# SciSharp/Gym.NET

Hardware: AMD Instinct MI355X
Metric: env-steps/sec (higher is better)
Workload: dtype f32

## Files before the change

### gym.net_amd/csrc/envs.hpp

```cpp
#pragma once
#include <hip/hip_runtime.h>
#include <stdint.h>

#include "philox.hpp"

namespace gymnet {


typedef float f2 __attribute__((ext_vector_type(2)));
namespace vm {
__device__ __forceinline__ float splat(float, float v) { return v; }
__device__ __forceinline__ f2 splat(f2, float v) { return f2{v, v}; }
__device__ __forceinline__ float fma(float a, float b, float c) { return fmaf(a, b, c); }
__device__ __forceinline__ f2 fma(f2 a, f2 b, f2 c) { return __builtin_elementwise_fma(a, b, c); }
template <class T> __device__ __forceinline__ T fmak(float k, T b, T c) { return fma(splat(b, k), b, c); }
template <class T> __device__ __forceinline__ T fmac(T a, T b, float k) { return fma(a, b, splat(a, k)); }
}

__device__ __forceinline__ void sincos_quadrant(float s, float c, float n, float &s_out, float &c_out) {
    const uint32_t q = (uint32_t)(int)n;
    const uint32_t q30 = q << 30, q31 = q << 31;
    const bool odd = (int32_t)q31 < 0;
    const float ss = odd ? c : s, cc = odd ? s : c;
    s_out = __uint_as_float(__builtin_amdgcn_bitop3_b32(__float_as_uint(ss), q30, 0x80000000u, 0x78));
// ... 39 lines not shown
    T ps = vm::fmac(vm::splat(z, -1.9515295891e-4f), z, 8.3321608736e-3f);
    ps = vm::fmac(ps, z, -1.6666654611e-1f);
    const T s = vm::fma(r * z, ps, r);
    T pc = vm::fmac(vm::splat(z, 2.443315711809948e-5f), z, -1.388731625493765e-3f);
    pc = vm::fmac(pc, z, 4.166664568298827e-2f);
    pc = vm::fmac(pc, z, -0.5f);
    const T c = vm::fmac(pc, z, 1.0f);
    if constexpr (sizeof(T) == sizeof(float)) {
        sincos_quadrant(s, c, n, s_out, c_out);
    } else {
        float s0, c0, s1, c1;
        sincos_quadrant(s.x, c.x, n.x, s0, c0);
        sincos_quadrant(s.y, c.y, n.y, s1, c1);
        s_out = T{s0, s1};
        c_out = T{c0, c1};
    }
}

constexpr float kSmallAngle = 0.785f;
__device__ __forceinline__ void sincos_tiny(float x, float &s_out, float &c_out) {
    const float z = x * x;
    float ps = fmaf(-1.9515295891e-4f, z, 8.3321608736e-3f);
    ps = fmaf(ps, z, -1.6666654611e-1f);
    s_out = fmaf(x * z, ps, x);
    float pc = fmaf(2.443315711809948e-5f, z, -1.388731625493765e-3f);
    pc = fmaf(pc, z, 4.166664568298827e-2f);
    c_out = fmaf(z * z, pc, fmaf(-0.5f, z, 1.0f));
}

template <bool BOUNDED = false>
__device__ __forceinline__ void sincos_f32(float x, float &s_out, float &c_out) {
    if constexpr (!BOUNDED) {
        if (__builtin_expect(fabsf(x) > 65536.0f, 0)) {
            sincosf(x, &s_out, &c_out);
            return;
        }
    }
    sincos_bounded<float>(x, s_out, c_out);
}
__device__ __forceinline__ float sin_f32(float x) { float s, c; sincos_f32(x, s, c); return s; }
__device__ __forceinline__ float cos_f32(float x) { float s, c; sincos_f32(x, s, c); return c; }

template <typename Dummy = void>
struct DivByTotalMass {
    static constexpr float C = 0.1f + 1.0f;
    static constexpr float ZH = 1.0f / C;
    static constexpr float ZL = (float)(1.0 / (double)C - (double)ZH);
    __device__ __forceinline__ static float apply(float x) { return fmaf(x, ZH, x * ZL); }
};

struct CartPole {
    static constexpr int S = 4;
    static constexpr int O = 4;
    static constexpr bool OBS_ALIASES_STATE = true;
    static constexpr bool HAS_SBD = true;
    static constexpr bool BOX_ACTION = false;
    static constexpr bool PACKED2 = false;
    static constexpr bool PIPE_LANES = false, PIPE_PAIRS = false;
    using Action = int32_t;
    using Real = float;
    static constexpr bool RESET_TAKES_KEY = false;
    static constexpr const char *NAME = "CartPole";
    static constexpr int32_t ACTION_N = 2;

    static constexpr float gravity = 9.8f;
    static constexpr float masspole = 0.1f;
    static constexpr float total_mass = 0.1f + 1.0f;
    static constexpr float length = 0.5f;
    static constexpr float polemass_length = 0.1f * 0.5f;
    static constexpr float force_mag = 10.0f;
    static constexpr float tau = 0.02f;
    static constexpr float theta_threshold = 0.20943951606750488f;
    static constexpr float x_threshold = 2.4f;

    __device__ __forceinline__ static float div_tm(float x) { return DivByTotalMass<>::apply(x); }

    static constexpr bool HAS_SMALL_ANGLE_PATH = true;
    static constexpr int ANGLE_ROW = 2;
    static constexpr float SMALL_ANGLE_BOUND = kSmallAngle;

    template <bool SMALL_ANGLE = false, bool AUTORESET = false>
    __device__ __forceinline__ static void step(float (&s)[S], Action a, float &reward, bool &done) {
        const float x = s[0], x_dot = s[1], theta = s[2], theta_dot = s[3];
        const float force = (a == 1) ? force_mag : -force_mag;
        float sintheta, costheta;
        if constexpr (SMALL_ANGLE) sincos_tiny(theta, sintheta, costheta);
        else sincos_f32(theta, sintheta, costheta);
        const float temp = div_tm(force + polemass_length * theta_dot * theta_dot * sintheta);
        const float thetaacc = (gravity * sintheta - costheta * temp)
                               / (length * (4.0f / 3.0f - div_tm(masspole * costheta * costheta)));
        const float xacc = temp - div_tm(polemass_length * thetaacc * costheta);
        const float nx = x + tau * x_dot;
        const float nx_dot = x_dot + tau * xacc;
        const float ntheta = theta + tau * theta_dot;
        const float ntheta_dot = theta_dot + tau * thetaacc;
        s[0] = nx; s[1] = nx_dot; s[2] = ntheta; s[3] = ntheta_dot;
        const double vx = __builtin_fma((double)tau, (double)x_dot, (double)x);
        const double vtheta = __builtin_fma((double)tau, (double)theta_dot, (double)theta);
        done = __builtin_fabs(vx) > (double)x_threshold || __builtin_fabs(vtheta) > (double)theta_threshold;
        reward = 1.0f;
    }

    __device__ __forceinline__ static void reset(float (&s)[S], const PhiloxWords &r) {
#pragma unroll
        for (int k = 0; k < 4; ++k) s[k] = -0.05f + 0.1f * u01_24(r.w[k]);
    }

    __device__ __forceinline__ static void observe(const float (&s)[S], float (&o)[O]) {
#pragma unroll
        for (int k = 0; k < 4; ++k) o[k] = s[k];
    }
    __device__ __forceinline__ static void observe_fresh(const float (&s)[S], float (&o)[O]) { observe(s, o); }
    __device__ __forceinline__ static void step_observe(float (&s)[S], Action a, float &reward, bool &done, float (&o)[O]) {
        step(s, a, reward, done);
        observe(s, o);
    }
};

struct Pendulum {
    static constexpr int S = 2;
    static constexpr int O = 3;
    static constexpr bool OBS_ALIASES_STATE = false;
    static constexpr int OBS_ROW_OF_STATE[S] = {-1, 2};
    static constexpr bool HAS_SBD = false;
    static constexpr bool BOX_ACTION = true;
    static constexpr bool PACKED2 = false;
    static constexpr bool PIPE_LANES = false, PIPE_PAIRS = false;
    static constexpr bool HAS_SMALL_ANGLE_PATH = false;
    using Action = float;
    using Real = float;
    static constexpr bool RESET_TAKES_KEY = false;
    static constexpr const char *NAME = "Pendulum";
    static constexpr float ACTION_LOW = -2.0f, ACTION_HIGH = 2.0f;
    static constexpr float PI = 3.14159265358979323846f;

    __device__ __forceinline__ static float fmod_2pi(float a) {
        constexpr float m = 2.0f * PI, inv_m = 1.0f / m;
        const float ax = fabsf(a);
        if (__builtin_expect(!(ax < 4194304.0f * m), 0)) return fmodf(a, m);
        float q = truncf(ax * inv_m);
        float r = fmaf(-q, m, ax);
        q = r < 0.0f ? q - 1.0f : (r >= m ? q + 1.0f : q);
        r = fmaf(-q, m, ax);
        return copysignf(r, a);
    }

    __device__ __forceinline__ static float floored_mod_2pi(float a) {
        float r = fmod_2pi(a);
        if (r < 0.0f) r += 2.0f * PI;
        return r;
    }

    __device__ __forceinline__ static void step(float (&s)[S], Action a, float &reward, bool &done) {
        const float max_speed = 8.0f, max_torque = 2.0f, dt = 0.05f;
        const float th = s[0], thdot = s[1];
        const float u = a < -max_torque ? -max_torque : (a > max_torque ? max_torque : a);
        const float nrm = floored_mod_2pi(th + PI) - PI;
        const float costs = nrm * nrm + 0.1f * (thdot * thdot) + 0.001f * (u * u);
        float newthdot = thdot + (15.0f * sin_f32(th) + 3.0f * u) * dt;
        newthdot = newthdot < -max_speed ? -max_speed : (newthdot > max_speed ? max_speed : newthdot);
        const float newth = th + newthdot * dt;
        s[0] = newth; s[1] = newthdot;
        reward = -costs;
        done = false;
    }

    __device__ __forceinline__ static void reset(float (&s)[S], const PhiloxWords &r) {
        s[0] = -PI + (2.0f * PI) * u01_24(r.w[0]);
        s[1] = -1.0f + 2.0f * u01_24(r.w[1]);
    }

    __device__ __forceinline__ static void observe(const float (&s)[S], float (&o)[O]) {
        float sn, cs;
        sincos_f32(s[0], sn, cs);
        o[0] = cs; o[1] = sn; o[2] = s[1];
    }
    __device__ __forceinline__ static void observe_fresh(const float (&s)[S], float (&o)[O]) { observe(s, o); }
    __device__ __forceinline__ static void step_observe(float (&s)[S], Action a, float &reward, bool &done, float (&o)[O]) {
        step(s, a, reward, done);
        observe(s, o);
    }
};

// ... 225 lines not shown
```

### gym.net_amd/csrc/lanes.hpp

```cpp
#pragma once
#include <hip/hip_runtime.h>
#include <stdint.h>

namespace gymnet {

template <class T, int N> struct VecOf { typedef T type __attribute__((ext_vector_type(N))); };
typedef float f32x4 __attribute__((ext_vector_type(4)));
typedef int32_t i32x4 __attribute__((ext_vector_type(4)));

template <class T, int VEC>
constexpr int piece_of() { return (int)(16 / sizeof(T)) < VEC ? (int)(16 / sizeof(T)) : VEC; }

template <class T, int VEC, bool NT, bool GUARD>
__device__ __forceinline__ void load_row(const T *__restrict__ p, int64_t i0, int64_t n, T (&v)[VEC]) {
    if constexpr (VEC > 1 && sizeof(T) > 1) {
        if (!GUARD || i0 + VEC <= n) {
            constexpr int P = piece_of<T, VEC>();
            static_assert(VEC % P == 0, "VEC must be a whole number of 16-byte pieces");
            typedef typename VecOf<T, P>::type V;
#pragma unroll
            for (int q = 0; q < VEC / P; ++q) {
                V t;
                if constexpr (NT) t = __builtin_nontemporal_load(reinterpret_cast<const V *>(p + i0 + q * P));
                else t = *reinterpret_cast<const V *>(p + i0 + q * P);
#pragma unroll
                for (int j = 0; j < P; ++j) v[q * P + j] = t[j];
            }
            return;
        }
    }
#pragma unroll
    for (int j = 0; j < VEC; ++j) {
        if (!GUARD || i0 + j < n) { if constexpr (NT) v[j] = __builtin_nontemporal_load(p + i0 + j); else v[j] = p[i0 + j]; }
        else v[j] = T(0);
    }
}

template <class T, int VEC, bool NT, bool GUARD>
__device__ __forceinline__ void store_row(T *__restrict__ p, int64_t i0, int64_t n, const T (&v)[VEC]) {
    if constexpr (VEC > 1 && sizeof(T) > 1) {
        if (!GUARD || i0 + VEC <= n) {
            constexpr int P = piece_of<T, VEC>();
            static_assert(P == 2 || P == 4, "16-byte pieces of 4- or 8-byte elements");
            typedef typename VecOf<T, P>::type V;
#pragma unroll
            for (int q = 0; q < VEC / P; ++q) {
                V t;
                if constexpr (P == 4) t = V{v[q * P], v[q * P + 1], v[q * P + 2], v[q * P + 3]};
                else t = V{v[q * P], v[q * P + 1]};
#ifdef GYMNET_PROBE_STORE_SC1
                if constexpr (NT && sizeof(T) == 4 && P == 4) {
                    asm volatile("global_store_dwordx4 %0, %1, off sc1" :: "v"(p + i0 + q * P), "v"(t) : "memory");
                    continue;
                }
#endif
                if constexpr (NT) __builtin_nontemporal_store(t, reinterpret_cast<V *>(p + i0 + q * P));
                else *reinterpret_cast<V *>(p + i0 + q * P) = t;
            }
            return;
        }
    }
#pragma unroll
    for (int j = 0; j < VEC; ++j)
        if (!GUARD || i0 + j < n) { if constexpr (NT) __builtin_nontemporal_store(v[j], p + i0 + j); else p[i0 + j] = v[j]; }
}

template <int VEC, bool NT, bool GUARD>
__device__ __forceinline__ void store_u8(uint8_t *__restrict__ p, int64_t i0, int64_t n, const uint8_t (&v)[VEC]) {
    if constexpr (VEC == 2) {
        if (!GUARD || i0 + 2 <= n) {
            const uint16_t w = (uint16_t)((uint16_t)v[0] | ((uint16_t)v[1] << 8));
            if constexpr (NT) __builtin_nontemporal_store(w, reinterpret_cast<uint16_t *>(p + i0));
            else *reinterpret_cast<uint16_t *>(p + i0) = w;
            return;
        }
    }
    if constexpr (VEC == 4) {
        if (!GUARD || i0 + 4 <= n) {
            const uint32_t w = (uint32_t)v[0] | ((uint32_t)v[1] << 8) | ((uint32_t)v[2] << 16) | ((uint32_t)v[3] << 24);
            if constexpr (NT) __builtin_nontemporal_store(w, reinterpret_cast<uint32_t *>(p + i0));
            else *reinterpret_cast<uint32_t *>(p + i0) = w;
            return;
        }
    }
#pragma unroll
    for (int j = 0; j < VEC; ++j)
        if (!GUARD || i0 + j < n) { if constexpr (NT) __builtin_nontemporal_store(v[j], p + i0 + j); else p[i0 + j] = v[j]; }
}

template <int VEC, bool NT, bool GUARD>
__device__ __forceinline__ void load_f32(const float *__restrict__ p, int64_t i0, int64_t n, float (&v)[VEC]) { load_row<float, VEC, NT, GUARD>(p, i0, n, v); }
template <int VEC, bool NT, bool GUARD>
__device__ __forceinline__ void store_f32(float *__restrict__ p, int64_t i0, int64_t n, const float (&v)[VEC]) { store_row<float, VEC, NT, GUARD>(p, i0, n, v); }
template <int VEC, bool NT, bool GUARD>
__device__ __forceinline__ void load_i32(const int32_t *__restrict__ p, int64_t i0, int64_t n, int32_t (&v)[VEC]) { load_row<int32_t, VEC, NT, GUARD>(p, i0, n, v); }
template <int VEC, bool NT, bool GUARD>
__device__ __forceinline__ void store_i32(int32_t *__restrict__ p, int64_t i0, int64_t n, const int32_t (&v)[VEC]) { store_row<int32_t, VEC, NT, GUARD>(p, i0, n, v); }

__device__ __forceinline__ uint32_t lane_id() {
    return __builtin_amdgcn_mbcnt_hi(~0u, __builtin_amdgcn_mbcnt_lo(~0u, 0u));
}

}
```

### gym.net_amd/csrc/step_kernels.hpp

```cpp
#pragma once
#include "kernels.hpp"

#include <cstdio>
#include <type_traits>

#include "lanes.hpp"
#include "philox.hpp"

namespace gymnet {

__device__ __forceinline__ float abs_real(float x) { return fabsf(x); }
__device__ __forceinline__ double abs_real(double x) { return __builtin_fabs(x); }

template <class Env, bool UNIFORM_KEY = false>
__device__ __forceinline__ void draw_reset(typename Env::Real (&s)[Env::S], uint64_t key, uint64_t lane, uint64_t tick) {
    if constexpr (Env::RESET_TAKES_KEY) Env::reset(s, key, lane, tick);
    else Env::reset(s, lane_words<UNIFORM_KEY>(key, lane, tick));
}

template <class Env>
__device__ __forceinline__ constexpr bool state_row_own(int k) {
    if constexpr (Env::OBS_ALIASES_STATE) return true; else return Env::OBS_ROW_OF_STATE[k] < 0;
}
template <class Env>
__device__ __forceinline__ const typename Env::Real *state_row_src(const typename Env::Real *state, int64_t state_stride,
                                                                    const typename Env::Real *obs_in, int64_t obs_stride, int k) {
    if constexpr (Env::OBS_ALIASES_STATE) return state + k * state_stride;
    else return Env::OBS_ROW_OF_STATE[k] < 0 ? state + k * state_stride : obs_in + Env::OBS_ROW_OF_STATE[k] * obs_stride;
}

__device__ __forceinline__ uint32_t wave_shard() {
    return (uint32_t)((((int64_t)blockIdx.x * blockDim.x + threadIdx.x) >> 6) & (kShards - 1));
}

template <int VEC, class Args>
__device__ __forceinline__ void count_after_done(const Args &a, const bool (&after)[VEC]) {
    uint32_t total = 0;
#pragma unroll
    for (int j = 0; j < VEC; ++j) total += (uint32_t)__popcll(__ballot(after[j]));
    if (total && lane_id() == (uint32_t)(__ffsll((unsigned long long)__ballot(1)) - 1))
        atomicAdd(&a.after_done[wave_shard() * kAfterStride], (unsigned long long)total);
}

template <class Env, bool AUTORESET, bool SMALL_ANGLE = false>
__device__ __forceinline__ void advance_sublane(typename Env::Real (&sj)[Env::S], typename Env::Action act, int32_t &sbd, float &rw,
                                                bool &dn, bool &after, bool in_range, typename Env::Real (&oj)[Env::O]) {
    if constexpr (Env::HAS_SMALL_ANGLE_PATH) Env::template step<SMALL_ANGLE, AUTORESET>(sj, act, rw, dn);
    else if constexpr (Env::OBS_ALIASES_STATE) Env::step(sj, act, rw, dn);
    else Env::step_observe(sj, act, rw, dn, oj);
    if constexpr (!AUTORESET && Env::HAS_SBD) {
        if (dn) {
            if (sbd == -1) { sbd = 0; }
            else { after = in_range; sbd += 1; rw = 0.0f; }
        }
    }
}

template <class Env, int VEC>
__device__ __forceinline__ bool wave_angles_small(const typename Env::Real (&s)[Env::S][VEC]) {
    if constexpr (!Env::HAS_SMALL_ANGLE_PATH) return false;
    else {
        bool small = true;
#pragma unroll
        for (int j = 0; j < VEC; ++j) small = small && (abs_real(s[Env::ANGLE_ROW][j]) <= Env::SMALL_ANGLE_BOUND);
        return __ballot(!small) == 0;
    }
}

template <class Env, int VEC, bool AUTORESET, bool GUARD, bool PACK = true>
__device__ __forceinline__ void advance_all(typename Env::Real (&s)[Env::S][VEC], typename Env::Action (&act)[VEC], int32_t (&sbd)[VEC],
                                            float (&rw)[VEC], bool (&dn)[VEC], bool (&after)[VEC], typename Env::Real (&o)[Env::O][VEC],
                                            int64_t i0, int64_t n) {
    constexpr int S = Env::S, O = Env::O;
    using Real = typename Env::Real;
#ifndef GYMNET_PROBE_NO_PACK
    constexpr bool kPack = true;
#else
    constexpr bool kPack = false;
#endif
    if constexpr (Env::PACKED2 && VEC == 2 && kPack && PACK) {
        Env::step_observe_x2(s, act, rw, dn, o);
    } else {
        auto all_sublanes = [&](auto small_tag) {
#pragma unroll
            for (int j = 0; j < VEC; ++j) {
                Real sj[S], oj[O];
#pragma unroll
                for (int k = 0; k < S; ++k) sj[k] = s[k][j];
                advance_sublane<Env, AUTORESET, decltype(small_tag)::value>(sj, act[j], sbd[j], rw[j], dn[j], after[j], !GUARD || i0 + j < n, oj);
#pragma unroll
                for (int k = 0; k < S; ++k) s[k][j] = sj[k];
                if constexpr (!Env::OBS_ALIASES_STATE) {
#pragma unroll
                    for (int k = 0; k < O; ++k) o[k][j] = oj[k];
                }
            }
        };
        if constexpr (Env::HAS_SMALL_ANGLE_PATH) {
            if (wave_angles_small<Env, VEC>(s)) all_sublanes(std::true_type{});
            else all_sublanes(std::false_type{});
        } else {
            all_sublanes(std::false_type{});
        }
    }
}

template <class Env, int VEC, bool LANE_SEEDS>
__device__ __forceinline__ void reset_pending(uint32_t pending, typename Env::Real (&s)[Env::S][VEC], typename Env::Real (&o)[Env::O][VEC],
                                              const StepArgsT<typename Env::Real> &a, int64_t i0, int64_t n, uint64_t tick) {
    constexpr int S = Env::S, O = Env::O;
    using Real = typename Env::Real;
    while (pending) {
        const int j = __ffs(pending) - 1;
        pending &= pending - 1;
        Real sj[S];
        bool drawn = false;
        if constexpr (LANE_SEEDS) {
            if (a.lane_seed) {
                draw_reset<Env, false>(sj, i0 + j < n ? a.lane_seed[i0 + j] : a.seed, a.lane_offset + (uint64_t)(i0 + j), tick);
                drawn = true;
            }
        }
        if (!drawn) draw_reset<Env, true>(sj, a.seed, a.lane_offset + (uint64_t)(i0 + j), tick);
        Real oj[O];
        if constexpr (!Env::OBS_ALIASES_STATE) Env::observe_fresh(sj, oj);
#pragma unroll
        for (int jj = 0; jj < VEC; ++jj) {
            if (jj == j) {
#pragma unroll
                for (int k = 0; k < S; ++k) s[k][jj] = sj[k];
                if constexpr (!Env::OBS_ALIASES_STATE) {
#pragma unroll
                    for (int k = 0; k < O; ++k) o[k][jj] = oj[k];
                }
            }
        }
    }
}

template <class Env>
constexpr bool has_split_reset() { return Env::RESET_TAKES_KEY && Env::OBS_ALIASES_STATE; }

__device__ __forceinline__ PhiloxWords neighbour_words(const PhiloxWords &w) {
    PhiloxWords o;
#pragma unroll
    for (int k = 0; k < 4; ++k) o.w[k] = (uint32_t)__builtin_amdgcn_mov_dpp((int)w.w[k], 0xB1, 0xF, 0xF, true);
    return o;
}

#ifdef GYMNET_PROBE_RESET_MASKED
constexpr bool kResetFullExec = false;
#else
constexpr bool kResetFullExec = true;
#endif

template <class Env>
struct ResetScratch {
    uint32_t slot[64];
    typename Env::Real draw[64][Env::S];
};

__device__ __forceinline__ void wave_lds_fence() {
    __builtin_amdgcn_fence(__ATOMIC_RELEASE, "wavefront");
    __builtin_amdgcn_wave_barrier();
    __builtin_amdgcn_fence(__ATOMIC_ACQUIRE, "wavefront");
}

template <class Env, int VEC, bool LANE_SEEDS>
__device__ __forceinline__ void reset_pending_wave(uint32_t pending, typename Env::Real (&s)[Env::S][VEC], const StepArgsT<typename Env::Real> &a,
                                                   int64_t i0, int64_t n, uint64_t tick, ResetScratch<Env> *sc) {
    constexpr int S = Env::S;
    using Real = typename Env::Real;
    static_assert(Env::OBS_ALIASES_STATE, "the compacted reset hands back the state only");
    const uint32_t lane = lane_id();
    uint32_t rank[VEC];
    uint32_t total = 0;
#pragma unroll
    for (int j = 0; j < VEC; ++j) {
        const uint64_t m = __ballot((pending >> j) & 1u);
        rank[j] = total + __builtin_amdgcn_mbcnt_hi((uint32_t)(m >> 32), __builtin_amdgcn_mbcnt_lo((uint32_t)m, 0u));
        total += (uint32_t)__popcll(m);
    }
    if (total == 0) return;
    const int64_t wave_i0 = i0 - (int64_t)lane * VEC;
    constexpr bool SPLIT = has_split_reset<Env>();
    const uint32_t active = (uint32_t)__popcll(__ballot(1));
    const uint32_t A = SPLIT ? active >> 1 : active;
    if constexpr (SPLIT) {
        if (A == 0) {
            Real o_unused[Env::O][VEC];
            reset_pending<Env, VEC, LANE_SEEDS>(pending, s, o_unused, a, i0, n, tick);
            return;
        }
    }
    for (uint32_t base = 0; base < total; base += A) {
#pragma unroll
        for (int j = 0; j < VEC; ++j)
            if (((pending >> j) & 1u) && rank[j] - base < A) sc->slot[rank[j] - base] = lane * VEC + (uint32_t)j;
        wave_lds_fence();
        if constexpr (SPLIT) {
            const uint32_t r = lane >> 1, call = lane & 1u;
            const bool draws = r < A && r < total - base;
            PhiloxWords w{};
            if (kResetFullExec || draws) {
                const uint32_t sl = sc->slot[draws ? r : 0u];
                const int64_t gl = wave_i0 + (int64_t)sl;
                uint64_t key = a.seed;
                if constexpr (LANE_SEEDS) {
                    if (a.lane_seed && gl < n) key = a.lane_seed[gl];
                }
                w = lane_words(Env::reset_call_key(key, call), a.lane_offset + (uint64_t)gl, tick);
            }
            const PhiloxWords other = neighbour_words(w);
            if ((kResetFullExec || draws) && call == 0) {
                Real sj[S];
                Env::reset_from_words(sj, w, other);
#pragma unroll
                for (int k = 0; k < S; ++k) sc->draw[r][k] = sj[k];
            }
        } else if (kResetFullExec || lane < total - base) {
            const uint32_t sl = sc->slot[lane < total - base ? lane : 0u];
            const int64_t gl = wave_i0 + (int64_t)sl;
            Real sj[S];
            bool drawn = false;
            if constexpr (LANE_SEEDS) {
                if (a.lane_seed) {
                    draw_reset<Env, false>(sj, gl < n ? a.lane_seed[gl] : a.seed, a.lane_offset + (uint64_t)gl, tick);
                    drawn = true;
                }
            }
            if (!drawn) draw_reset<Env, true>(sj, a.seed, a.lane_offset + (uint64_t)gl, tick);
#pragma unroll
            for (int k = 0; k < S; ++k) sc->draw[lane][k] = sj[k];
        }
        wave_lds_fence();
        Real got[VEC][S];
#pragma unroll
        for (int j = 0; j < VEC; ++j) {
            const uint32_t r = rank[j] - base;
#pragma unroll
            for (int k = 0; k < S; ++k) got[j][k] = sc->draw[r < A ? r : 0u][k];
        }
#pragma unroll
        for (int j = 0; j < VEC; ++j) {
            const bool mine = ((pending >> j) & 1u) && rank[j] - base < A;
#pragma unroll
            for (int k = 0; k < S; ++k) s[k][j] = mine ? got[j][k] : s[k][j];
        }
        wave_lds_fence();
    }
}

template <int VEC>
__device__ __forceinline__ uint32_t rank_finished(const bool (&finished)[VEC], uint32_t (&off)[VEC]) {
    uint32_t total = 0;
#pragma unroll
    for (int j = 0; j < VEC; ++j) {
        const uint64_t m = __ballot(finished[j]);
        off[j] = total + __builtin_amdgcn_mbcnt_hi((uint32_t)(m >> 32), __builtin_amdgcn_mbcnt_lo((uint32_t)m, 0u));
        total += (uint32_t)__popcll(m);
    }
    return total;
}

template <class Env, int VEC>
__device__ __forceinline__ void append_done_records(const StepArgsT<typename Env::Real> &a, const bool (&finished)[VEC], int64_t i0,
                                                    const typename Env::Real (&s)[Env::S][VEC], const typename Env::Real (&o)[Env::O][VEC],
                                                    const float (&fin_ret)[VEC], const int32_t (&fin_len)[VEC], bool stats) {
    constexpr int S = Env::S, O = Env::O;
    const uint32_t lane = lane_id();
    uint32_t off[VEC];
    const uint32_t total = rank_finished<VEC>(finished, off);
    if (total) {
        const int leader = __ffsll((unsigned long long)__ballot(1)) - 1;
        const uint32_t shard = wave_shard();
        uint32_t base = 0;
        if ((int)lane == leader)
            base = atomicAdd(&a.done_count2[a.cparity * (kShards * kCountStride) + shard * kCountStride], total);
        base = __shfl(base, leader);
        const int64_t seg0 = (int64_t)shard * a.done_cap;
#pragma unroll
        for (int j = 0; j < VEC; ++j) {
            if (!finished[j]) continue;
            const int64_t pos = seg0 + base + off[j];
            a.done_list[pos] = (int32_t)(i0 + j);
            if (stats) { a.rec_ret[pos] = fin_ret[j]; a.rec_len[pos] = fin_len[j]; }
            if (a.rec_obs) {
#pragma unroll
                for (int k = 0; k < O; ++k)
                    a.rec_obs[((int64_t)shard * O + k) * a.done_cap + base + off[j]] = Env::OBS_ALIASES_STATE ? s[k < S ? k : 0][j] : o[k][j];
            }
        }
    }
}

template <class R>
__device__ __forceinline__ StepArgsT<R> hot_step_args(R *state, const void *action, int64_t n, int64_t state_stride, uint64_t *tick2, float *reward,
                                                      int32_t parity, const StepArgsT<R> &rest) {
    StepArgsT<R> a = rest;
    a.state = state; a.action = action; a.n = n; a.state_stride = state_stride; a.tick2 = tick2; a.reward = reward; a.parity = parity;
    return a;
}

template <class Env, int VEC>
struct LaneInputs {
    typename Env::Real s[Env::S][VEC];
    typename Env::Action act[VEC];
    int32_t sbd[VEC];
};

template <bool NT, class T>
__device__ __forceinline__ T load_elem(const T *p) { if constexpr (NT) return __builtin_nontemporal_load(p); else return *p; }

template <class T, int VEC, bool NT>
__device__ __forceinline__ void load_row_clamped(const T *__restrict__ p, int64_t i0, int64_t n, T (&v)[VEC]) {
#pragma unroll
    for (int j = 0; j < VEC; ++j) v[j] = load_elem<NT>(p + (i0 + j < n ? i0 + j : n - 1));
}

template <class Env, int VEC, bool AUTORESET, int NT>
__device__ __forceinline__ void load_inputs_clamped(const StepArgsT<typename Env::Real> &a, const int64_t i0, LaneInputs<Env, VEC> &in) {
    constexpr bool NT_SL = (NT & 1) != 0, NT_A = (NT & 4) != 0;
#pragma unroll
    for (int k = 0; k < Env::S; ++k)
        load_row_clamped<typename Env::Real, VEC, NT_SL>(state_row_src<Env>(a.state, a.state_stride, a.obs_in, a.obs_stride, k), i0, a.n, in.s[k]);
    if constexpr (Env::BOX_ACTION) load_row_clamped<float, VEC, NT_A>(static_cast<const float *>(a.action), i0, a.n, in.act);
    else load_row_clamped<int32_t, VEC, NT_A>(static_cast<const int32_t *>(a.action), i0, a.n, in.act);
#pragma unroll
    for (int j = 0; j < VEC; ++j) in.sbd[j] = 0;
    if constexpr (!AUTORESET && Env::HAS_SBD) load_row_clamped<int32_t, VEC, NT_SL>(a.sbd, i0, a.n, in.sbd);
}

template <class Env, int VEC, bool AUTORESET, int NT, bool GUARD>
// ... 32 lines not shown
            if constexpr (GUARD) { load_row_clamped<float, VEC, NT_SL>(a.ep_ret, i0, n, ep_ret); load_row_clamped<int32_t, VEC, NT_SL>(a.ep_len, i0, n, ep_len); }
            else { load_f32<VEC, NT_SL, false>(a.ep_ret, i0, n, ep_ret); load_i32<VEC, NT_SL, false>(a.ep_len, i0, n, ep_len); }
        }
#pragma unroll
        for (int j = 0; j < VEC; ++j) { fin_ret[j] = 0.0f; fin_len[j] = 0; }
    }

    float reward[VEC];
    uint8_t done[VEC];
    bool finished[VEC];
    bool after[VEC];
#pragma unroll
    for (int j = 0; j < VEC; ++j) after[j] = false;
    Real o[O][VEC];
    uint32_t pending = 0;

    float rwv[VEC];
    bool dnv[VEC];
    advance_all<Env, VEC, AUTORESET, GUARD, PACK>(s, act, sbd, rwv, dnv, after, o, i0, n);

#pragma unroll
    for (int j = 0; j < VEC; ++j) {
        const float rw = rwv[j];
        uint8_t db = dnv[j] ? 1 : 0;
        if constexpr (EXTRAS) {
            if (stats) {
                ep_ret[j] += rw;
                ep_len[j] += 1;
                if (a.max_episode_steps > 0 && ep_len[j] >= a.max_episode_steps) db |= 2;
            }
        }
        const bool fin = db != 0;
        finished[j] = fin && (!GUARD || i0 + j < n);
        done[j] = db;
        reward[j] = rw;

        if constexpr (EXTRAS) {
            if (fin && a.final_obs && (!GUARD || i0 + j < n)) {
#pragma unroll
                for (int k = 0; k < O; ++k) a.final_obs[k * n + i0 + j] = Env::OBS_ALIASES_STATE ? s[k < S ? k : 0][j] : o[k][j];
            }
            if (stats && fin && (!GUARD || i0 + j < n)) {
                fin_ret[j] = ep_ret[j];
                fin_len[j] = ep_len[j];
                if (a.fin_ret) { a.fin_ret[i0 + j] = ep_ret[j]; a.fin_len[i0 + j] = ep_len[j]; }
                if constexpr (AUTORESET) { ep_ret[j] = 0.0f; ep_len[j] = 0; }
            }
        }

        if constexpr (AUTORESET) pending |= fin ? (1u << j) : 0u;
    }

    if constexpr (!AUTORESET && Env::HAS_SBD) count_after_done<VEC>(a, after);

    store_f32<VEC, NT_O, GUARD>(a.reward, i0, n, reward);
    store_u8<VEC, NT_O, GUARD>(a.done, i0, n, done);

    if constexpr (EXTRAS) {
        if (a.done_list) append_done_records<Env, VEC>(a, finished, i0, s, o, fin_ret, fin_len, stats);
    }

    if constexpr (AUTORESET && RESETF == 1) reset_pending_wave<Env, VEC, EXTRAS>(pending, s, a, i0, n, tick, sc);
    else if constexpr (AUTORESET) reset_pending<Env, VEC, EXTRAS>(pending, s, o, a, i0, n, tick);

#pragma unroll
    for (int k = 0; k < S; ++k)
        if (state_row_own<Env>(k)) store_row<Real, VEC, NT_SS, GUARD>(a.state_out + k * a.state_stride, i0, n, s[k]);
    if constexpr (!Env::OBS_ALIASES_STATE) {
#pragma unroll
        for (int k = 0; k < O; ++k) store_row<Real, VEC, NT_SS, GUARD>(a.obs + k * a.obs_stride, i0, n, o[k]);
    }
    if constexpr (!AUTORESET && Env::HAS_SBD) store_i32<VEC, NT_SS, GUARD>(a.sbd, i0, n, sbd);

    if constexpr (EXTRAS) {
        if (stats) { store_f32<VEC, NT_SS, GUARD>(a.ep_ret, i0, n, ep_ret); store_i32<VEC, NT_SS, GUARD>(a.ep_len, i0, n, ep_len); }
    }
}

template <class Env, int VEC, bool AUTORESET, bool EXTRAS, int NT, bool GUARD, int RESETF = 0>
__device__ __forceinline__ void step_body(const StepArgsT<typename Env::Real> &a, const int64_t i0, const uint64_t tick, ResetScratch<Env> *sc = nullptr) {
    LaneInputs<Env, VEC> in;
    load_inputs<Env, VEC, AUTORESET, NT, GUARD>(a, i0, in);
    advance_and_store<Env, VEC, AUTORESET, EXTRAS, NT, GUARD, RESETF>(a, i0, tick, in, sc);
}

template <class Env>
struct LaneOutputs { typename Env::Real s[Env::S], o[Env::O]; float reward; uint8_t done; int32_t sbd; };

template <class Env, bool AUTORESET>
__device__ __forceinline__ void compute_lane(const StepArgsT<typename Env::Real> &a, int64_t i, uint64_t tick, LaneInputs<Env, 1> &in,
                                             LaneOutputs<Env> &out) {
    constexpr int S = Env::S, O = Env::O;
    typename Env::Real o[O][1];
    float rw[1];
    bool dn[1], after[1] = {false};
    advance_all<Env, 1, AUTORESET, false>(in.s, in.act, in.sbd, rw, dn, after, o, i, a.n);
    if constexpr (!AUTORESET && Env::HAS_SBD) count_after_done<1>(a, after);
    if constexpr (AUTORESET) reset_pending<Env, 1, false>(dn[0] ? 1u : 0u, in.s, o, a, i, a.n, tick);
#pragma unroll
    for (int k = 0; k < S; ++k) out.s[k] = in.s[k][0];
#pragma unroll
    for (int k = 0; k < O; ++k) out.o[k] = o[k][0];
    out.reward = rw[0]; out.done = dn[0] ? 1 : 0; out.sbd = in.sbd[0];
}

template <class Env, bool AUTORESET, int NT>
__device__ __forceinline__ void store_lane(const StepArgsT<typename Env::Real> &a, int64_t i, const LaneOutputs<Env> &out) {
    constexpr bool NT_SS = (NT & 2) != 0, NT_O = (NT & 8) != 0;
    auto st = [](auto *p, auto v, bool nt) { if (nt) __builtin_nontemporal_store(v, p); else *p = v; };
    st(a.reward + i, out.reward, NT_O);
    if constexpr (NT_O) __builtin_nontemporal_store(out.done, a.done + i); else a.done[i] = out.done;
#pragma unroll
    for (int k = 0; k < Env::S; ++k)
        if (state_row_own<Env>(k)) st(a.state_out + k * a.state_stride + i, out.s[k], NT_SS);
    if constexpr (!Env::OBS_ALIASES_STATE) {
#pragma unroll
        for (int k = 0; k < Env::O; ++k) st(a.obs + k * a.obs_stride + i, out.o[k], NT_SS);
    }
    if constexpr (!AUTORESET && Env::HAS_SBD) a.sbd[i] = out.sbd;
}

template <class Env, int ITEMS, bool AUTORESET, int NT>
__global__ __launch_bounds__(256) void step_kernel_pipe(typename Env::Real *state, const void *action, int64_t n, int64_t state_stride, uint64_t *tick2,
                                                        float *reward, int32_t block, int32_t parity, const StepArgsT<typename Env::Real> rest) {
    const StepArgsT<typename Env::Real> a = hot_step_args(state, action, n, state_stride, tick2, reward, parity, rest);
    const uint64_t tick = a.tick2[a.parity];
    if (blockIdx.x == 0 && threadIdx.x == 0) a.tick2[a.parity ^ 1] = tick + 1;
    const int64_t T = (int64_t)gridDim.x * block;
    const int64_t i = (int64_t)blockIdx.x * block + threadIdx.x;
    LaneInputs<Env, 1> in[ITEMS];
#pragma unroll
    for (int k = 0; k < ITEMS; ++k) {
        const int64_t idx = i + k * T;
        load_inputs<Env, 1, AUTORESET, NT, false>(a, idx < a.n ? idx : a.n - 1, in[k]);
    }
#pragma unroll
    for (int k = 0; k < ITEMS; ++k) {
        LaneOutputs<Env> out;
        if (k == 0) {
#pragma unroll
            for (int c = 0; c < Env::S; ++c) asm volatile("" : "+v"(in[0].s[c][0]));
            asm volatile("" : "+v"(in[0].act[0]));
        }
        compute_lane<Env, AUTORESET>(a, i + k * T, tick, in[k], out);
        if (k == 0) {
#pragma unroll
            for (int kk = 1; kk < ITEMS; ++kk) {
#pragma unroll
                for (int c = 0; c < Env::S; ++c) asm volatile("" : "+v"(in[kk].s[c][0]), "+v"(out.s[Env::S - 1]));
                asm volatile("" : "+v"(in[kk].act[0]), "+v"(out.reward));
            }
        }
        if (i + k * T < a.n) store_lane<Env, AUTORESET, NT>(a, i + k * T, out);
    }
}

template <class Env>
struct DeferScratch {
    uint32_t slot[32];
    typename Env::Real draw[32][Env::S];
};

template <class Env, int PAIRS, class StateOf>
__device__ __forceinline__ void reset_group_deferred(uint32_t pending, StateOf s, const StepArgsT<typename Env::Real> &a, int64_t t_wave0,
                                                     int64_t T, int first_pair, uint64_t tick, DeferScratch<Env> *sc) {
    static_assert(Env::RESET_CALLS == 2 && 2 * PAIRS <= 8, "two lanes per reset; the slot word keeps 3 bits for the sub-lane position");
// ... 146 lines not shown
    static_assert(std::is_same<typename Env::Real, float>::value, "the producer / consumer form stages float rows through LDS");
    constexpr int kLdsComputeWaves = CW, kLdsTile = CW * 64;
    constexpr int S = Env::S, O = Env::O;
    constexpr int NOWN = own_state_rows<Env>();
    constexpr int NROW = NOWN + (Env::OBS_ALIASES_STATE ? 0 : O) + 1;
    constexpr bool NT_SS = (NT & 2) != 0, NT_O = (NT & 8) != 0;
    __shared__ float out_buf[2][NROW][kLdsTile];
    __shared__ uint8_t done_buf[2][kLdsTile];
    const uint64_t tick = a.tick2[a.parity];
    if (blockIdx.x == 0 && threadIdx.x == 0) a.tick2[a.parity ^ 1] = tick + 1;
    const int lane = threadIdx.x & 63;
    const bool storer = (threadIdx.x >> 6) == kLdsComputeWaves;
    const int cl = threadIdx.x;
    const int64_t t0 = (int64_t)blockIdx.x * TPB;
    const int nt = (int)(tiles - t0 < TPB ? tiles - t0 : TPB);

    auto tile_barrier = [] { asm volatile("s_waitcnt lgkmcnt(0)\n\ts_barrier" ::: "memory"); };

    LaneInputs<Env, 1> in[TPB + 1];
    if (!storer) load_inputs<Env, 1, AUTORESET, NT, false>(a, t0 * kLdsTile + cl, in[0]);
#pragma unroll
    for (int s = 0; s <= TPB; ++s) {
        if (!storer) {
            if (s < TPB) {
                const int64_t i = (t0 + (s < nt ? s : nt - 1)) * kLdsTile + cl;
                const int64_t ip = (t0 + (s + 1 < nt ? s + 1 : nt - 1)) * kLdsTile + cl;
                load_inputs<Env, 1, AUTORESET, NT, false>(a, ip, in[s + 1]);
#pragma unroll
                for (int c = 0; c < S; ++c) asm volatile("" : "+v"(in[s].s[c][0]));
                asm volatile("" : "+v"(in[s].act[0]));
                LaneOutputs<Env> out;
                compute_lane<Env, AUTORESET>(a, i, tick, in[s], out);
#pragma unroll
                for (int c = 0; c < S; ++c) asm volatile("" : "+v"(in[s + 1].s[c][0]), "+v"(out.s[S - 1]));
                asm volatile("" : "+v"(in[s + 1].act[0]), "+v"(out.reward));
                if (s < nt) {
                    int r = 0;
#pragma unroll
                    for (int k = 0; k < S; ++k)
                        if (state_row_own<Env>(k)) out_buf[s & 1][r++][cl] = out.s[k];
                    if constexpr (!Env::OBS_ALIASES_STATE) {
#pragma unroll
                        for (int k = 0; k < O; ++k) out_buf[s & 1][r++][cl] = out.o[k];
                    }
                    out_buf[s & 1][r][cl] = out.reward;
                    done_buf[s & 1][cl] = out.done;
                }
            }
        } else if (s >= 1 && s - 1 < nt) {
            const int b = (s - 1) & 1;
            const int64_t base = (t0 + s - 1) * kLdsTile;
            auto drain = [&](float *row, int r, bool nt_store) {
#pragma unroll
                for (int j = 0; j < kLdsTile / 256; ++j) {
                    const f32x4 v = *reinterpret_cast<const f32x4 *>(&out_buf[b][r][j * 256 + lane * 4]);
                    f32x4 *dst = reinterpret_cast<f32x4 *>(row + base + j * 256 + lane * 4);
                    if (nt_store) __builtin_nontemporal_store(v, dst); else *dst = v;
                }
                static_assert(kLdsTile % 256 == 0, "the storing wave moves 256 floats per instruction");
            };
            int r = 0;
#pragma unroll
            for (int k = 0; k < S; ++k)
                if (state_row_own<Env>(k)) drain(a.state_out + k * a.state_stride, r++, NT_SS);
            if constexpr (!Env::OBS_ALIASES_STATE) {
#pragma unroll
                for (int k = 0; k < O; ++k) drain(a.obs + k * a.obs_stride, r++, NT_SS);
            }
            drain(a.reward, r, NT_O);
            if (lane < kLdsTile / 16) {
                const i32x4 v = *reinterpret_cast<const i32x4 *>(&done_buf[b][lane * 16]);
                i32x4 *dst = reinterpret_cast<i32x4 *>(a.done + base + lane * 16);
                if constexpr (NT_O) __builtin_nontemporal_store(v, dst); else *dst = v;
            }
        }
        tile_barrier();
    }
}

template <class Env, int VEC, bool AUTORESET, bool EXTRAS, int NT, int RESETF = 0>
__global__ __launch_bounds__(256) void step_kernel(typename Env::Real *state, const void *action, int64_t n, int64_t state_stride, uint64_t *tick2,
                                                   float *reward, int32_t block, int32_t parity, const StepArgsT<typename Env::Real> rest) {
    const StepArgsT<typename Env::Real> a = hot_step_args(state, action, n, state_stride, tick2, reward, parity, rest);
    const int64_t i0 = ((int64_t)blockIdx.x * block + threadIdx.x) * VEC;
    ResetScratch<Env> *sc = nullptr;
    if constexpr (RESETF == 1) {
        __shared__ ResetScratch<Env> scratch[256 / 64];
        sc = &scratch[threadIdx.x >> 6];
    }
    const uint64_t tick = a.tick2[a.parity];
    if (blockIdx.x == 0 && threadIdx.x == 0) {
        a.tick2[a.parity ^ 1] = tick + 1;
    }
    if constexpr (EXTRAS) {
        if (blockIdx.x == 0 && a.done_count2)
            for (int sh = threadIdx.x; sh < kShards; sh += block) a.done_count2[(a.cparity ^ 1) * (kShards * kCountStride) + sh * kCountStride] = 0u;
    }
    if (((int64_t)blockIdx.x + 1) * block * VEC <= a.n) {
        step_body<Env, VEC, AUTORESET, EXTRAS, NT, false, RESETF>(a, i0, tick, sc);
    } else {
        if (i0 >= a.n) return;
        step_body<Env, VEC, AUTORESET, EXTRAS, NT, true, RESETF>(a, i0, tick, sc);
    }
}

template <class Env>
__device__ __forceinline__ typename Env::Action sampled_action(uint32_t word_a) {
    if constexpr (Env::BOX_ACTION) return Env::ACTION_LOW + (Env::ACTION_HIGH - Env::ACTION_LOW) * u01_24(word_a);
    else return (int32_t)__umulhi(word_a, (uint32_t)Env::ACTION_N);
}

template <int VEC>
__device__ __forceinline__ void thread_action_words(uint64_t seed, uint64_t gl0, uint64_t tick, bool want_aux, bool one_group,
                                                    uint32_t (&wa)[VEC], uint32_t (&wb)[VEC]) {
    static_assert(VEC == 1 || VEC == 2 || VEC == 4, "a thread's lanes must fit one group of four");
    if (one_group) {
        const PhiloxWords r = action_group_words<true>(seed, gl0 >> 2, tick);
        PhiloxWords c{};
        if (want_aux) c = aux_group_words<true>(seed, gl0 >> 2, tick);
        const uint32_t base = (uint32_t)gl0 & 3u;
        if constexpr (VEC == 4) {
#pragma unroll
            for (int j = 0; j < 4; ++j) { wa[j] = r.w[j]; wb[j] = c.w[j]; }
        } else if constexpr (VEC == 2) {
#pragma unroll
            for (int j = 0; j < 2; ++j) { wa[j] = base ? r.w[2 + j] : r.w[j]; wb[j] = base ? c.w[2 + j] : c.w[j]; }
        } else {
            wa[0] = word_of(r, base); wb[0] = word_of(c, base);
        }
    } else {
#pragma unroll
        for (int j = 0; j < VEC; ++j) { wa[j] = 0u; wb[j] = 0u; }
#pragma unroll 1
        for (int j = 0; j < VEC; ++j) {
            const uint32_t a = action_word<true>(seed, gl0 + (uint64_t)j, tick);
            const uint32_t b = want_aux ? aux_word<true>(seed, gl0 + (uint64_t)j, tick) : 0u;
#pragma unroll
            for (int k = 0; k < VEC; ++k) { wa[k] = k == j ? a : wa[k]; wb[k] = k == j ? b : wb[k]; }
        }
    }
}

constexpr uint32_t kStageRecords = 256;
struct EpisodeStage { int32_t t[kStageRecords], lane[kStageRecords]; float ret[kStageRecords]; int32_t len[kStageRecords]; };

struct NoHook { static constexpr bool CHOOSES = false; };

struct NoRepeat { static constexpr bool ON = false; };
struct HeldAction { static constexpr bool ON = true; int32_t R; };

template <class Env, int VEC, bool AUTORESET, bool GUARD, bool EXTRAS, bool SAMPLE, int RESETF = 0, int RECORDS = 0, class Hook = NoHook, class Rep = NoRepeat>
__device__ __forceinline__ void rollout_body(const StepArgsT<typename Env::Real> &a, const RolloutArgsT<typename Env::Real> &ro,
                                             const int64_t i0, const uint64_t tick0, ResetScratch<Env> *sc = nullptr, EpisodeStage *stage = nullptr,
                                             Hook hook = Hook{}, Rep rep = Rep{}) {
    static_assert(!Rep::ON || (!Hook::CHOOSES && !(Env::PACKED2 && VEC == 2)), "frame skip: ring / sampled actions, unpacked sub-lanes");
    constexpr int S = Env::S, O = Env::O;
    using Act = typename Env::Action;
    using Real = typename Env::Real;
    const int64_t n = a.n;

    Real s[S][VEC];
#pragma unroll
    for (int k = 0; k < S; ++k) load_row<Real, VEC, true, GUARD>(state_row_src<Env>(a.state, a.state_stride, a.obs_in, a.obs_stride, k), i0, n, s[k]);
    int32_t sbd[VEC] = {};
    if constexpr (!AUTORESET && Env::HAS_SBD) load_i32<VEC, true, GUARD>(a.sbd, i0, n, sbd);

    auto load_action = [&](int64_t slice, Act (&dst)[VEC]) {
        const char *base = static_cast<const char *>(a.action) + (size_t)(slice * ro.action_stride) * 4;
        if constexpr (Env::BOX_ACTION) load_f32<VEC, true, GUARD>(reinterpret_cast<const float *>(base), i0, n, dst);
        else load_i32<VEC, true, GUARD>(reinterpret_cast<const int32_t *>(base), i0, n, dst);
    };

    Act act[VEC], act_next[VEC];
    bool use_ring = true;
    const bool one_group = (a.lane_offset % (uint64_t)VEC) == 0;
    const uint32_t explore_at_or_below = coin_threshold(ro.epsilon);
    if constexpr (SAMPLE && !Hook::CHOOSES) {
        use_ring = ro.action_source == 2;
#pragma unroll
        for (int j = 0; j < VEC; ++j) { act[j] = Act(0); act_next[j] = Act(0); }
        if (use_ring) load_action(0, act);
    } else if constexpr (!Hook::CHOOSES) {
// ... 593 lines not shown
```

Baseline: 159.0 billion.

## Add full-workgroup CartPole step body with wave-uniform addressing and late done ballot

Adds a specialised step body for full workgroups of autoreset, small-angle-capable envs like CartPole. Row bases become wave-uniform scalar pointers with 32-bit per-lane offsets, which trims 64-bit address arithmetic. Termination is computed afterwards from the saved input state, and its ballot masks drive a compacted per-wave reset through LDS. Together these aim to cut VALU and address overhead per step, at the cost of more code paths and extra register pressure from keeping the old state.

```diff
diff --git a/gym.net_amd/csrc/envs.hpp b/gym.net_amd/csrc/envs.hpp
--- a/gym.net_amd/csrc/envs.hpp
+++ b/gym.net_amd/csrc/envs.hpp
@@ -145,6 +145,7 @@
     template <bool SMALL_ANGLE = false, bool AUTORESET = false>
     __device__ __forceinline__ static void step(float (&s)[S], Action a, float &reward, bool &done) {
         const float x = s[0], x_dot = s[1], theta = s[2], theta_dot = s[3];
+        const float s_in[S] = {x, x_dot, theta, theta_dot};
         const float force = (a == 1) ? force_mag : -force_mag;
         float sintheta, costheta;
         if constexpr (SMALL_ANGLE) sincos_tiny(theta, sintheta, costheta);
@@ -158,10 +159,18 @@
         const float ntheta = theta + tau * theta_dot;
         const float ntheta_dot = theta_dot + tau * thetaacc;
         s[0] = nx; s[1] = nx_dot; s[2] = ntheta; s[3] = ntheta_dot;
-        const double vx = __builtin_fma((double)tau, (double)x_dot, (double)x);
-        const double vtheta = __builtin_fma((double)tau, (double)theta_dot, (double)theta);
-        done = __builtin_fabs(vx) > (double)x_threshold || __builtin_fabs(vtheta) > (double)theta_threshold;
+        bool term[DONE_TERMS];
+        done_terms_of_inputs(s_in, term);
+        done = term[0] || term[1];
         reward = 1.0f;
+    }
+
+    static constexpr int DONE_TERMS = 2;
+    __device__ __forceinline__ static void done_terms_of_inputs(const float (&s)[S], bool (&term)[DONE_TERMS]) {
+        const double vx = __builtin_fma((double)tau, (double)s[1], (double)s[0]);
+        const double vtheta = __builtin_fma((double)tau, (double)s[3], (double)s[2]);
+        term[0] = __builtin_fabs(vx) > (double)x_threshold;
+        term[1] = __builtin_fabs(vtheta) > (double)theta_threshold;
     }
 
     __device__ __forceinline__ static void reset(float (&s)[S], const PhiloxWords &r) {
diff --git a/gym.net_amd/csrc/lanes.hpp b/gym.net_amd/csrc/lanes.hpp
--- a/gym.net_amd/csrc/lanes.hpp
+++ b/gym.net_amd/csrc/lanes.hpp
@@ -1,6 +1,8 @@
 #pragma once
 #include <hip/hip_runtime.h>
 #include <stdint.h>
+
+#include <type_traits>
 
 namespace gymnet {
 
@@ -88,6 +90,67 @@
         if (!GUARD || i0 + j < n) { if constexpr (NT) __builtin_nontemporal_store(v[j], p + i0 + j); else p[i0 + j] = v[j]; }
 }
 
+struct WgLanes {
+    int64_t first;
+    uint32_t local;
+};
+
+template <class T>
+__device__ __forceinline__ T *wave_uniform(T *p) {
+    const uint64_t u = reinterpret_cast<uint64_t>(p);
+    const uint32_t lo = __builtin_amdgcn_readfirstlane((uint32_t)u), hi = __builtin_amdgcn_readfirstlane((uint32_t)(u >> 32));
+    typedef __attribute__((address_space(1))) T *G;
+    return (T *)reinterpret_cast<G>(((uint64_t)hi << 32) | lo);
+}
+
+__device__ __forceinline__ uint32_t reissued(uint32_t x) { asm volatile("" : "+v"(x)); return x; }
+
+template <class V, class T>
+__device__ __forceinline__ V *wg_elem(T *row, uint32_t local, int extra) {
+    typedef typename std::conditional<std::is_const<T>::value, const char, char>::type B;
+    return reinterpret_cast<V *>(reinterpret_cast<B *>(row) + (uint32_t)(local * (uint32_t)sizeof(T)) + extra * (int)sizeof(T));
+}
+
+template <class T, int VEC, bool NT>
+__device__ __forceinline__ void load_row_wg(const T *__restrict__ row, uint32_t local, T (&v)[VEC]) {
+    constexpr int P = VEC > 1 ? piece_of<T, VEC>() : 1;
+    typedef typename std::conditional<(P > 1), typename VecOf<T, (P > 1 ? P : 2)>::type, T>::type V;
+#pragma unroll
+    for (int q = 0; q < VEC / P; ++q) {
+        const V *p = wg_elem<const V>(row, local, q * P);
+        V t;
+        if constexpr (NT) t = __builtin_nontemporal_load(p); else t = *p;
+        if constexpr (P > 1) {
+#pragma unroll
+            for (int j = 0; j < P; ++j) v[q * P + j] = t[j];
+        } else v[q] = t;
+    }
+}
+
+template <class T, int VEC, bool NT>
+__device__ __forceinline__ void store_row_wg(T *__restrict__ row, uint32_t local, const T (&v)[VEC]) {
+    constexpr int P = VEC > 1 ? piece_of<T, VEC>() : 1;
+    static_assert(P == 1 || P == 2 || P == 4, "16-byte pieces of 4- or 8-byte elements");
+    typedef typename std::conditional<(P > 1), typename VecOf<T, (P > 1 ? P : 2)>::type, T>::type V;
+#pragma unroll
+    for (int q = 0; q < VEC / P; ++q) {
+        V *p = wg_elem<V>(row, local, q * P);
+        V t;
+        if constexpr (P == 4) t = V{v[q * P], v[q * P + 1], v[q * P + 2], v[q * P + 3]};
+        else if constexpr (P == 2) t = V{v[q * P], v[q * P + 1]};
+        else t = v[q];
+        if constexpr (NT) __builtin_nontemporal_store(t, p); else *p = t;
+    }
+}
+
+template <int VEC, bool NT>
+__device__ __forceinline__ void store_done_word_wg(uint8_t *__restrict__ row, uint32_t local, uint32_t w) {
+    static_assert(VEC == 1 || VEC == 2 || VEC == 4, "a done word is 1, 2 or 4 bytes");
+    typedef typename std::conditional<VEC == 4, uint32_t, typename std::conditional<VEC == 2, uint16_t, uint8_t>::type>::type W;
+    W *p = wg_elem<W>(row, local, 0);
+    if constexpr (NT) __builtin_nontemporal_store((W)w, p); else *p = (W)w;
+}
+
 template <int VEC, bool NT, bool GUARD>
 __device__ __forceinline__ void load_f32(const float *__restrict__ p, int64_t i0, int64_t n, float (&v)[VEC]) { load_row<float, VEC, NT, GUARD>(p, i0, n, v); }
 template <int VEC, bool NT, bool GUARD>
diff --git a/gym.net_amd/csrc/step_kernels.hpp b/gym.net_amd/csrc/step_kernels.hpp
--- a/gym.net_amd/csrc/step_kernels.hpp
+++ b/gym.net_amd/csrc/step_kernels.hpp
@@ -105,6 +105,52 @@
     }
 }
 
+template <class Env, class = void> struct has_done_of_inputs : std::false_type {};
+template <class Env> struct has_done_of_inputs<Env, std::void_t<decltype(&Env::done_terms_of_inputs)>> : std::true_type {};
+
+template <class Env, int VEC, bool AUTORESET>
+__device__ __forceinline__ void advance_all_late_done(typename Env::Real (&s)[Env::S][VEC], typename Env::Action (&act)[VEC], float (&rw)[VEC],
+                                                      bool (&dn)[VEC], uint64_t (&dmask)[VEC]) {
+    constexpr int S = Env::S, O = Env::O;
+    using Real = typename Env::Real;
+    static_assert(Env::HAS_SMALL_ANGLE_PATH && Env::OBS_ALIASES_STATE && has_done_of_inputs<Env>::value, "see above");
+    static_assert(AUTORESET || !Env::HAS_SBD, "the steps_beyond_done rule reads the flag inside the step");
+    Real was[S][VEC];
+#pragma unroll
+    for (int k = 0; k < S; ++k)
+#pragma unroll
+        for (int j = 0; j < VEC; ++j) was[k][j] = s[k][j];
+    auto all_sublanes = [&](auto small_tag) {
+#pragma unroll
+        for (int j = 0; j < VEC; ++j) {
+            Real sj[S], oj[O];
+            int32_t sbd_unused = 0;
+            bool after_unused = false;
+#pragma unroll
+            for (int k = 0; k < S; ++k) sj[k] = s[k][j];
+            advance_sublane<Env, AUTORESET, decltype(small_tag)::value>(sj, act[j], sbd_unused, rw[j], dn[j], after_unused, true, oj);
+#pragma unroll
+            for (int k = 0; k < S; ++k) s[k][j] = sj[k];
+        }
+    };
+    if (wave_angles_small<Env, VEC>(s)) all_sublanes(std::true_type{});
+    else all_sublanes(std::false_type{});
+#pragma unroll
+    for (int j = 0; j < VEC; ++j) {
+        Real wj[S];
+#pragma unroll
+        for (int k = 0; k < S; ++k) wj[k] = was[k][j];
+        bool term[Env::DONE_TERMS];
+        Env::done_terms_of_inputs(wj, term);
+        bool any = false;
+        uint64_t m = 0;
+#pragma unroll
+        for (int q = 0; q < Env::DONE_TERMS; ++q) { any = any || term[q]; m |= __builtin_amdgcn_ballot_w64(term[q]); }
+        dn[j] = any;
+        dmask[j] = m;
+    }
+}
+
 template <class Env, int VEC, bool LANE_SEEDS>
 __device__ __forceinline__ void reset_pending(uint32_t pending, typename Env::Real (&s)[Env::S][VEC], typename Env::Real (&o)[Env::O][VEC],
                                               const StepArgsT<typename Env::Real> &a, int64_t i0, int64_t n, uint64_t tick) {
@@ -249,6 +295,64 @@
         }
         wave_lds_fence();
     }
+}
+
+template <class Env, int VEC, bool LANE_SEEDS>
+__device__ __forceinline__ void reset_finished_wave(const bool (&fin)[VEC], const uint64_t (&fmask)[VEC], typename Env::Real (&s)[Env::S][VEC], const StepArgsT<typename Env::Real> &a,
+                                                    int64_t i0, int64_t wave_i0, int64_t n, uint64_t tick, ResetScratch<Env> *sc) {
+    constexpr int S = Env::S;
+    using Real = typename Env::Real;
+    static_assert(Env::OBS_ALIASES_STATE && !has_split_reset<Env>(), "one-call resets that hand back the state only");
+    const uint32_t lane = lane_id();
+    uint32_t rank[VEC];
+    uint32_t total = 0;
+#pragma unroll
+    for (int j = 0; j < VEC; ++j) {
+        const uint64_t m = fmask[j];
+        rank[j] = total + __builtin_amdgcn_mbcnt_hi((uint32_t)(m >> 32), __builtin_amdgcn_mbcnt_lo((uint32_t)m, 0u));
+        total += (uint32_t)__popcll(m);
+    }
+    if (__builtin_expect(total == 0 || total > 64u || __ballot(1) != ~0ull, 0)) {
+        if (total != 0) {
+            uint32_t pending = 0;
+#pragma unroll
+            for (int j = 0; j < VEC; ++j) pending |= fin[j] ? (1u << j) : 0u;
+            reset_pending_wave<Env, VEC, LANE_SEEDS>(pending, s, a, i0, n, tick, sc);
+        }
+        return;
+    }
+#pragma unroll
+    for (int j = 0; j < VEC; ++j)
+        if (fin[j]) sc->slot[rank[j]] = lane * VEC + (uint32_t)j;
+    wave_lds_fence();
+    {
+        const uint32_t sl = sc->slot[lane < total ? lane : 0u];
+        const int64_t gl = wave_i0 + (int64_t)sl;
+        Real sj[S];
+        bool drawn = false;
+        if constexpr (LANE_SEEDS) {
+            if (a.lane_seed) {
+                draw_reset<Env, false>(sj, gl < n ? a.lane_seed[gl] : a.seed, a.lane_offset + (uint64_t)gl, tick);
+                drawn = true;
+            }
+        }
+        if (!drawn) draw_reset<Env, true>(sj, a.seed, a.lane_offset + (uint64_t)gl, tick);
+#pragma unroll
+        for (int k = 0; k < S; ++k) sc->draw[lane][k] = sj[k];
+    }
+    wave_lds_fence();
+    Real got[VEC][S];
+#pragma unroll
+    for (int j = 0; j < VEC; ++j) {
+#pragma unroll
+        for (int k = 0; k < S; ++k) got[j][k] = sc->draw[rank[j] & 63u][k];
+    }
+#pragma unroll
+    for (int j = 0; j < VEC; ++j) {
+#pragma unroll
+        for (int k = 0; k < S; ++k) s[k][j] = fin[j] ? got[j][k] : s[k][j];
+    }
+    wave_lds_fence();
 }
 
 template <int VEC>
@@ -447,6 +551,57 @@
     LaneInputs<Env, VEC> in;
     load_inputs<Env, VEC, AUTORESET, NT, GUARD>(a, i0, in);
     advance_and_store<Env, VEC, AUTORESET, EXTRAS, NT, GUARD, RESETF>(a, i0, tick, in, sc);
+}
+
+template <class Env, bool AUTORESET, bool EXTRAS>
+constexpr bool has_full_workgroup_body() {
+    return AUTORESET && !EXTRAS && Env::HAS_SMALL_ANGLE_PATH && Env::OBS_ALIASES_STATE && !has_split_reset<Env>() && has_done_of_inputs<Env>::value;
+}
+
+template <class T>
+__device__ __forceinline__ T *wg_row(T *row, const WgLanes &wg) { return wave_uniform(row + wg.first); }
+
+template <class Env, int VEC, int NT, int RESETF>
+__device__ __forceinline__ void step_body_wg(const StepArgsT<typename Env::Real> &a, const WgLanes wg, const uint64_t tick, ResetScratch<Env> *sc) {
+    constexpr int S = Env::S;
+    using Real = typename Env::Real;
+    constexpr bool NT_SL = (NT & 1) != 0, NT_SS = (NT & 2) != 0, NT_A = (NT & 4) != 0, NT_O = (NT & 8) != 0;
+    static_assert(!Env::BOX_ACTION && Env::OBS_ALIASES_STATE, "a discrete-action env whose observation is its state");
+    const int64_t i0 = wg.first + (int64_t)wg.local;
+
+    Real s[S][VEC];
+    typename Env::Action act[VEC];
+#pragma unroll
+    for (int k = 0; k < S; ++k) load_row_wg<Real, VEC, NT_SL>(wg_row(static_cast<const Real *>(a.state) + k * a.state_stride, wg), wg.local, s[k]);
+    load_row_wg<int32_t, VEC, NT_A>(wg_row(static_cast<const int32_t *>(a.action), wg), wg.local, act);
+
+    float reward[VEC];
+    bool finished[VEC];
+    uint64_t fmask[VEC];
+    advance_all_late_done<Env, VEC, true>(s, act, reward, finished, fmask);
+
+    {
+        const uint32_t local = reissued(wg.local);
+        store_row_wg<float, VEC, NT_O>(wg_row(a.reward, wg), local, reward);
+        uint32_t w = 0;
+#pragma unroll
+        for (int j = 0; j < VEC; ++j) w |= finished[j] ? (1u << (8 * j)) : 0u;
+        store_done_word_wg<VEC, NT_O>(wg_row(a.done, wg), local, w);
+    }
+
+    if constexpr (RESETF == 1) {
+        reset_finished_wave<Env, VEC, false>(finished, fmask, s, a, i0, wg.first + (int64_t)__builtin_amdgcn_readfirstlane(wg.local), a.n, tick, sc);
+    } else {
+        uint32_t pending = 0;
+#pragma unroll
+        for (int j = 0; j < VEC; ++j) pending |= finished[j] ? (1u << j) : 0u;
+        Real o_unused[Env::O][VEC];
+        reset_pending<Env, VEC, false>(pending, s, o_unused, a, i0, a.n, tick);
+    }
+
+    const uint32_t local = reissued(wg.local);
+#pragma unroll
+    for (int k = 0; k < S; ++k) store_row_wg<Real, VEC, NT_SS>(wg_row(a.state_out + k * a.state_stride, wg), local, s[k]);
 }
 
 template <class Env>
@@ -759,7 +914,8 @@
 __global__ __launch_bounds__(256) void step_kernel(typename Env::Real *state, const void *action, int64_t n, int64_t state_stride, uint64_t *tick2,
                                                    float *reward, int32_t block, int32_t parity, const StepArgsT<typename Env::Real> rest) {
     const StepArgsT<typename Env::Real> a = hot_step_args(state, action, n, state_stride, tick2, reward, parity, rest);
-    const int64_t i0 = ((int64_t)blockIdx.x * block + threadIdx.x) * VEC;
+    const WgLanes wg{(int64_t)blockIdx.x * block * VEC, (uint32_t)threadIdx.x * (uint32_t)VEC};
+    const int64_t i0 = wg.first + (int64_t)wg.local;
     ResetScratch<Env> *sc = nullptr;
     if constexpr (RESETF == 1) {
         __shared__ ResetScratch<Env> scratch[256 / 64];
@@ -774,7 +930,8 @@
             for (int sh = threadIdx.x; sh < kShards; sh += block) a.done_count2[(a.cparity ^ 1) * (kShards * kCountStride) + sh * kCountStride] = 0u;
     }
     if (((int64_t)blockIdx.x + 1) * block * VEC <= a.n) {
-        step_body<Env, VEC, AUTORESET, EXTRAS, NT, false, RESETF>(a, i0, tick, sc);
+        if constexpr (has_full_workgroup_body<Env, AUTORESET, EXTRAS>()) step_body_wg<Env, VEC, NT, RESETF>(a, wg, tick, sc);
+        else step_body<Env, VEC, AUTORESET, EXTRAS, NT, false, RESETF>(a, i0, tick, sc);
     } else {
         if (i0 >= a.n) return;
         step_body<Env, VEC, AUTORESET, EXTRAS, NT, true, RESETF>(a, i0, tick, sc);
```

New measurement: 163.5 billion (median of 6 runs). +2.8%, better.
